# KhutornoyYaroslav/vcm-ts

Measured on AMD Instinct MI355X. Metric: encoded frames/sec at 1920x1080 GOP-32, higher is better.
Workload: dtype f32 (fp16x3 split-MFMA, fp32 accumulate)

## Files before the change

### include/dcvc_hip.h

```cpp
#ifndef DCVC_HIP_H
#define DCVC_HIP_H

#include <stdint.h>

#ifdef __cplusplus
extern "C" {
#endif

#define DCVC_OK 0
#define DCVC_E_ARG (-1)
#define DCVC_E_LAUNCH (-2)
#define DCVC_E_RANGE (-3)

#define DCVC_STATUS_ACT_SATURATED 1

#define DCVC_MAX_SEG 3

#define DCVC_PREC_FP32 0
#define DCVC_PREC_FP16X3 1

typedef struct {
    const float *ptr;
    int32_t C;
    int32_t cs;
} dcvc_seg;

typedef struct {
    dcvc_seg seg[DCVC_MAX_SEG];
    int32_t nseg;
    int32_t N, Hin, Win;
    int32_t in_act;
    float in_slope;
    const float *wpack;
    const float *bpack;
    int32_t ks;
    int32_t stride;
    int32_t Cout;
    int32_t Cout_pad;
    float *out;
    int32_t out_cs;
    int32_t out_act;
    float out_slope;
    int32_t pixel_shuffle;
    const float *res;
    int32_t res_cs;
    const float *res_gate;
    const float *res2;
    int32_t res2_cs;
    int32_t precision;
    int32_t *status;
    float *chan_partial;
    int32_t tile_row0;
    int32_t tile_rows;
    int32_t pair_taps;
} dcvc_conv_args;

int32_t dcvc_conv_tile_rows(int32_t ks, int32_t stride);

int32_t dcvc_conv_chan_partial_parts(int32_t ks, int32_t stride, int32_t Hout, int32_t Wout);
int dcvc_channel_mean_finish(const float *chan_partial, int32_t parts, int32_t row_stride, float *mean, int32_t N,
                             int32_t C, int32_t HW, void *stream);

int64_t dcvc_conv_pack_size(int32_t Cout, int32_t ks, int32_t nseg, const int32_t *seg_C, int32_t *cout_pad);

int dcvc_conv_pack_weights(const float *w, const float *b, int32_t Cout, int32_t ks, int32_t nseg,
                           const int32_t *seg_C, int32_t pixel_shuffle, int32_t precision, float *wpack,
                           float *bpack);

int64_t dcvc_conv_pack_size_paired(int32_t Cout, int32_t Cin, int32_t *cout_pad);
int dcvc_conv_pack_weights_paired(const float *w, const float *b, int32_t Cout, int32_t Cin, float *wpack, float *bpack);

int dcvc_conv2d(const dcvc_conv_args *a, void *stream);

int64_t dcvc_conv_small_pack_bytes(int32_t Cout, int32_t ks, int32_t nseg, const int32_t *seg_C);
int dcvc_conv_small_pack_weights(const float *w, const float *b, int32_t Cout, int32_t ks, int32_t nseg,
                                 const int32_t *seg_C, void *wpack, float *bpack);
int dcvc_conv2d_small(const dcvc_conv_args *a, void *stream);

int64_t dcvc_conv_k32_pack_bytes(int32_t Cout, int32_t ks, int32_t nseg, const int32_t *seg_C, int32_t *cout_pad);
int dcvc_conv_k32_pack_weights(const float *w, const float *b, int32_t Cout, int32_t ks, int32_t nseg,
                               const int32_t *seg_C, int32_t pixel_shuffle, void *wpack, float *bpack);
int dcvc_conv2d_k32(const dcvc_conv_args *a, void *stream);
int dcvc_conv_k32_set_waves(int32_t waves);

int dcvc_warp(const float *src, int32_t src_cs, const float *flow, int32_t flow_cs, float *out, int32_t out_cs,
              int32_t N, int32_t H, int32_t W, int32_t C, void *stream);
int dcvc_up2(const float *src, int32_t src_cs, float *out, int32_t out_cs, float *out2, int32_t out2_cs,
             int32_t N, int32_t H, int32_t W, int32_t C, float scale, void *stream);
int dcvc_down2(const float *src, int32_t src_cs, float *out, int32_t out_cs, int32_t N, int32_t H, int32_t W,
               int32_t C, float scale, int32_t avgpool_order, void *stream);
int dcvc_maxpool2(const float *src, int32_t src_cs, float *out, int32_t out_cs, int32_t N, int32_t H, int32_t W,
                  int32_t C, void *stream);
int dcvc_copy_channels(const float *src, int32_t src_cs, float *out, int32_t out_cs, int64_t npix, int32_t C,
                       void *stream);
int dcvc_nchw_to_nhwc(const float *src, float *out, int32_t out_cs, int32_t N, int32_t C, int32_t H, int32_t W,
                      void *stream);
int dcvc_nhwc_to_nchw(const float *src, int32_t src_cs, float *out, int32_t N, int32_t C, int32_t H, int32_t W,
                      int32_t clamp01, void *stream);

int dcvc_channel_mean(const float *src, int32_t src_cs, float *mean, float *scratch, int32_t N, int32_t HW,
                      int32_t C, void *stream);
int dcvc_se_gate(const float *mean, const float *w1, const float *w2, float *gate, int32_t N, int32_t C,
                 int32_t Cr, void *stream);

int dcvc_scale_channels(const float *src, int32_t src_cs, float *out, int32_t out_cs, const float *q_basic,
// ... 60 lines not shown
```

### vcm_ts_amd/csrc/conv_mfma.hip

```cpp
#include <hip/hip_runtime.h>
#include <stdint.h>
#include <stdlib.h>
#include <string.h>
#include <vector>

#include "dcvc_hip.h"
#include "kernel_common.h"

namespace {

constexpr int LDK = 20;


struct ConvK {
    const float *seg_ptr[DCVC_MAX_SEG];
    int seg_C[DCVC_MAX_SEG];
    int seg_cs[DCVC_MAX_SEG];
    int nseg;
    int Hin, Win, Hout, Wout;
    int in_act;
    float in_slope;
    const float *wpack;
    const float *bpack;
    int Cout, Cout_pad;
    float *out;
    int out_cs;
    int out_act;
    float out_slope;
    int ps;
    const float *res;
    int res_cs;
    const float *res_gate;
    const float *res2;
    int res2_cs;
    int vec_epi;
    int *status;
    float *chan_partial;
    int ntx;
    int ty0, nty;
    int band_rows;
};

inline long dev_env_long(const char *name, long dflt) {
    const char *dev = getenv("DCVC_DEV");
    if (!dev || strcmp(dev, "1") != 0) return dflt;
    const char *v = getenv(name);
    return v ? atol(v) : dflt;
}


template <int KS, int S, int RPW, int NT, bool SPLIT, bool PAIR = false>
__global__ __launch_bounds__(256, 2) void conv_mfma(const ConvK a) {
    static_assert(!PAIR || (KS == 7 && S == 1 && SPLIT), "tap pairing is built for the 7x7 split-fp16 layers");
    constexpr int BH = 4 * RPW, BW = 32, BN = 32 * NT;
    constexpr int PH = (BH - 1) * S + KS, PW = (BW - 1) * S + KS, PAD = KS / 2;
    constexpr int T = PAIR ? KS * 4 : KS * KS;
    constexpr int TPS = PAIR ? 4 : (KS == 3 && S == 1) ? 9 : KS;
    constexpr int NST = T / TPS;
    constexpr int EPI_LD = BN + 4;
    constexpr int LDS_MAIN = PH * PW * LDK + TPS * 4 * BN * 4, LDS_EPI = 4 * 32 * EPI_LD, LDS_RED = 4 * BN;
    __shared__ __attribute__((aligned(16))) float lds[LDS_MAIN > LDS_EPI + LDS_RED ? LDS_MAIN : LDS_EPI + LDS_RED];
    float *patch = lds;
    float *wl = lds + PH * PW * LDK;

    const int tid = threadIdx.x, lane = tid & 63, wave = tid >> 6;
    const int nbn = a.Cout_pad / BN;
    const int nb = blockIdx.x % nbn, tx = blockIdx.x / nbn;
    if (tx >= a.ntx) return;
    const int ty = blockIdx.y + a.ty0;
    const int x0 = tx * BW, y0 = ty * BH, n0 = nb * BN, img = blockIdx.z;

    f32x16 acc[RPW][NT];
#pragma unroll
    for (int m = 0; m < RPW; ++m)
#pragma unroll
        for (int n = 0; n < NT; ++n)
#pragma unroll
            for (int r = 0; r < 16; ++r) acc[m][n][r] = 0.f;

    const int a_base = ((wave * RPW * S) * PW + (lane & 31) * S) * LDK + (lane >> 5) * 4;
    const int b_base = ((lane >> 5) * BN + (lane & 31)) * 4;
// ... 273 lines not shown
#pragma unroll
            for (int r = 0; r < 16; ++r) {
                const int ox = x0 + (r & 3) + 8 * (r >> 2) + 4 * hh;
                const size_t pix = a.ps ? ((size_t)(img * Ho + 2 * oy + dy) * Wo + 2 * ox + dx)
                                        : ((size_t)(img * Ho + oy) * Wo + ox);
                rv[r] = (a.res && ox < a.Wout) ? a.res[pix * a.res_cs + cf] : 0.f;
                rv2[r] = (a.res2 && ox < a.Wout) ? a.res2[pix * a.res2_cs + cf] : 0.f;
            }
#pragma unroll
            for (int r = 0; r < 16; ++r) {
                const int ox = x0 + (r & 3) + 8 * (r >> 2) + 4 * hh;
                if (ox >= a.Wout) continue;
                float v = acc[m][n][r] * inv_scale + bias;
                if (a.out_act == 1) v = act(v, a.out_slope);
                else if (a.out_act == 2) v = fminf(fmaxf(v, 0.f), 1.f);
                const size_t pix = a.ps ? ((size_t)(img * Ho + 2 * oy + dy) * Wo + 2 * ox + dx)
                                        : ((size_t)(img * Ho + oy) * Wo + ox);
                if (a.out_act == 3) {
                    const float mk = rv2[r] > 0.f ? 1.f : a.out_slope;
                    v = a.res ? __builtin_fmaf(v, mk, rv[r]) : v * mk;
                } else {
                    if (a.res) v = a.res_gate ? __builtin_fmaf(rv[r], gate, v) : v + rv[r];
                    if (a.res2) v = rv2[r] + v;
                }
                if (a.status) vmax = fmaxf(vmax, fabsf(v));
                a.out[pix * a.out_cs + cf] = v;
            }
        }
    }
    if (a.status && !(vmax <= ACT_LIMIT)) atomicOr(a.status, DCVC_STATUS_ACT_SATURATED);
}


template <int KS, int S, int RPW, int NT, bool PAIR = false>
int launch(ConvK &k, int N, hipStream_t st, int precision) {
    constexpr int BH = 4 * RPW, BN = 32 * NT;
    k.ntx = (k.Wout + 31) / 32;
    static const bool xcd_pad = dev_env_long("DCVC_XCD_PAD", 0) != 0;
    unsigned gx = (unsigned)(k.ntx * (k.Cout_pad / BN));
    if (xcd_pad && gx >= 8) gx = (gx + 7) & ~7u;
    k.nty = (k.Hout + BH - 1) / BH;
    if (k.ty0 < 0 || k.ty0 >= k.nty) return DCVC_E_ARG;
    const int rows = k.band_rows > 0 ? (k.band_rows < k.nty - k.ty0 ? k.band_rows : k.nty - k.ty0) : k.nty;
    dim3 grid(gx, (unsigned)rows, (unsigned)N);
    if (PAIR)
        hipLaunchKernelGGL((conv_mfma<KS, S, RPW, NT, true, PAIR>), grid, dim3(256), 0, st, k);
    else if (precision == DCVC_PREC_FP16X3)
        hipLaunchKernelGGL((conv_mfma<KS, S, RPW, NT, true>), grid, dim3(256), 0, st, k);
    else
        hipLaunchKernelGGL((conv_mfma<KS, S, RPW, NT, false>), grid, dim3(256), 0, st, k);
    RET_LAUNCH();
}

}

extern "C" int64_t dcvc_conv_pack_size(int32_t Cout, int32_t ks, int32_t nseg, const int32_t *seg_C, int32_t *cout_pad) {
    if (Cout <= 0 || nseg <= 0 || nseg > DCVC_MAX_SEG || (ks != 1 && ks != 3 && ks != 7)) return DCVC_E_ARG;
    int chunks = 0;
    for (int s = 0; s < nseg; ++s) chunks += (seg_C[s] + MFMA_KC - 1) / MFMA_KC;
    const int cp = round_up(Cout, 32);
    if (cout_pad) *cout_pad = cp;
    return (int64_t)chunks * ks * ks * 4 * cp * 4;
}

extern "C" int dcvc_conv_pack_weights(const float *w, const float *b, int32_t Cout, int32_t ks, int32_t nseg,
                                      const int32_t *seg_C, int32_t pixel_shuffle, int32_t precision, float *wpack,
                                      float *bpack) {
    if (precision != DCVC_PREC_FP32 && precision != DCVC_PREC_FP16X3) return DCVC_E_ARG;
    int32_t cp = 0;
    const int64_t total = dcvc_conv_pack_size(Cout, ks, nseg, seg_C, &cp);
    if (total < 0 || (pixel_shuffle && (Cout & 3))) return DCVC_E_ARG;
    const int T = ks * ks;
    int Cin = 0;
    for (int s = 0; s < nseg; ++s) Cin += seg_C[s];
    memset(wpack, 0, (size_t)total * sizeof(float));
    memset(bpack, 0, (size_t)cp * sizeof(float));
    const int Cq = Cout / 4;
    _Float16 *base = (_Float16 *)wpack;
    int cg = 0, cin0 = 0;
    for (int s = 0; s < nseg; ++s) {
        for (int c0 = 0; c0 < seg_C[s]; c0 += MFMA_KC, ++cg) {
            for (int t = 0; t < T; ++t)
// ... 29 lines not shown
    int32_t cp = 0;
    const int64_t total = dcvc_conv_pack_size_paired(Cout, Cin, &cp);
    if (total < 0 || !w || !wpack || !bpack) return DCVC_E_ARG;
    memset(wpack, 0, (size_t)total * sizeof(float));
    memset(bpack, 0, (size_t)cp * sizeof(float));
    _Float16 *base = (_Float16 *)wpack;
    bool clamped = false;
    for (int ky = 0; ky < 7; ++ky)
        for (int kx = 0; kx < 7; ++kx) {
            const int step = ky * 4 + (kx >> 1), h = kx & 1;
            for (int c = 0; c < Cin; ++c)
                for (int n = 0; n < Cout; ++n) {
                    float sv = w[((size_t)n * Cin + c) * 49 + ky * 7 + kx] * WGT_SCALE;
                    if (!(fabsf(sv) <= F16_MAX)) { clamped = true; sv = sv > 0.f ? F16_MAX : -F16_MAX; }
                    const SplitF16 p = split_f16(sv);
                    base[mfma_wpack_f16(0, 28, step, 8 * h + c, cp, n, 0)] = p.hi;
                    base[mfma_wpack_f16(0, 28, step, 8 * h + c, cp, n, 1)] = p.lo;
                }
        }
    for (int n = 0; n < Cout; ++n) bpack[n] = b ? b[n] : 0.f;
    return clamped ? DCVC_E_RANGE : DCVC_OK;
}

static int tile_rows(int ks, int stride) { return stride == 2 ? 4 : 8; }

extern "C" int32_t dcvc_conv_tile_rows(int32_t ks, int32_t stride) { return tile_rows(ks, stride); }

extern "C" int32_t dcvc_conv_chan_partial_parts(int32_t ks, int32_t stride, int32_t Hout, int32_t Wout) {
    if (Hout <= 0 || Wout <= 0 || (stride != 1 && stride != 2)) return DCVC_E_ARG;
    const int bh = tile_rows(ks, stride);
    return ((Wout + 31) / 32) * ((Hout + bh - 1) / bh);
}

extern "C" int dcvc_conv2d(const dcvc_conv_args *a, void *stream) {
    if (!conv_args_ok(a)) return DCVC_E_ARG;
    if (a->stride != 1 && a->stride != 2) return DCVC_E_ARG;
    if (a->precision != DCVC_PREC_FP32 && a->precision != DCVC_PREC_FP16X3) return DCVC_E_ARG;
    if (a->Cout_pad % 32 || a->Cout > a->Cout_pad || (a->pixel_shuffle && (a->Cout & 3))) return DCVC_E_ARG;
    if (a->out_act < 0 || a->out_act > 3) return DCVC_E_ARG;
    if (a->out_act == 3 && (!a->res2 || a->res_gate || a->chan_partial || a->pixel_shuffle)) return DCVC_E_ARG;
    ConvK k;
    memset(&k, 0, sizeof(k));
    copy_conv_args_full(k, a);
    k.Hin = a->Hin;
    k.Win = a->Win;
    const int pad = a->ks / 2;
    k.Hout = (a->Hin + 2 * pad - a->ks) / a->stride + 1;
    k.Wout = (a->Win + 2 * pad - a->ks) / a->stride + 1;
    k.vec_epi = vec_epilogue_ok(a);
    if (a->chan_partial && (!k.vec_epi || a->pixel_shuffle)) return DCVC_E_ARG;
    hipStream_t st = (hipStream_t)stream;
    const bool wide = (a->Cout_pad % 64) == 0;
    const int key = a->ks * 10 + a->stride;
    if (a->stride == 1 && !a->pair_taps && !a->chan_partial && a->tile_rows <= 0) {
        const long wgs8 = (long)((k.Wout + 31) / 32) * ((k.Hout + 7) / 8) * (a->Cout_pad / (wide ? 64 : 32)) * a->N;
        static const long rows4_below = dev_env_long("DCVC_ROWS4_WGS", 384);
        if (wgs8 < rows4_below) {
            if (a->ks == 3) return wide ? launch<3, 1, 1, 2>(k, a->N, st, a->precision) : launch<3, 1, 1, 1>(k, a->N, st, a->precision);
            if (a->ks == 7) return wide ? launch<7, 1, 1, 2>(k, a->N, st, a->precision) : launch<7, 1, 1, 1>(k, a->N, st, a->precision);
            if (a->ks == 1) return wide ? launch<1, 1, 1, 2>(k, a->N, st, a->precision) : launch<1, 1, 1, 1>(k, a->N, st, a->precision);
        }
    }
    switch (key) {
        case 11: return wide ? launch<1, 1, 2, 2>(k, a->N, st, a->precision) : launch<1, 1, 2, 1>(k, a->N, st, a->precision);
        case 12: return wide ? launch<1, 2, 1, 2>(k, a->N, st, a->precision) : launch<1, 2, 1, 1>(k, a->N, st, a->precision);
        case 31:
            return wide ? launch<3, 1, 2, 2>(k, a->N, st, a->precision) : launch<3, 1, 2, 1>(k, a->N, st, a->precision);
        case 32: return wide ? launch<3, 2, 1, 2>(k, a->N, st, a->precision) : launch<3, 2, 1, 1>(k, a->N, st, a->precision);
        case 71:
            if (a->pair_taps) {
                if (a->nseg != 1 || a->seg[0].C > 8 || a->precision != DCVC_PREC_FP16X3 || a->pixel_shuffle) return DCVC_E_ARG;
                return wide ? launch<7, 1, 2, 2, true>(k, a->N, st, a->precision) : launch<7, 1, 2, 1, true>(k, a->N, st, a->precision);
            }
            return wide ? launch<7, 1, 2, 2>(k, a->N, st, a->precision) : launch<7, 1, 2, 1>(k, a->N, st, a->precision);
        default: return DCVC_E_ARG;
    }
}
```

### vcm_ts_amd/csrc/conv_small.hip

```cpp
#include <hip/hip_runtime.h>
#include <stdint.h>
#include <string.h>

#include "dcvc_hip.h"
#include "kernel_common.h"

namespace {

constexpr int KC = 16;

struct SmallK {
    const float *seg_ptr[DCVC_MAX_SEG];
    int seg_C[DCVC_MAX_SEG];
    int seg_cs[DCVC_MAX_SEG];
    int nseg;
    int H, W;
    int in_act;
    float in_slope;
    const char *wpack;
    const float *bpack;
    int Cout;
    float *out;
    int out_cs, out_act;
    float out_slope;
// ... 185 lines not shown

extern "C" int dcvc_conv_small_pack_weights(const float *w, const float *b, int32_t Cout, int32_t ks, int32_t nseg,
                                            const int32_t *seg_C, void *wpack, float *bpack) {
    const int64_t total = dcvc_conv_small_pack_bytes(Cout, ks, nseg, seg_C);
    if (total < 0 || !w || !wpack || !bpack) return DCVC_E_ARG;
    const int T = ks * ks;
    int Cin = 0;
    for (int s = 0; s < nseg; ++s) Cin += seg_C[s];
    memset(wpack, 0, (size_t)total);
    for (int n = 0; n < 16; ++n) bpack[n] = (b && n < Cout) ? b[n] : 0.f;
    _Float16 *base = (_Float16 *)wpack;
    int status = DCVC_OK, cg = 0, cin0 = 0;
    for (int s = 0; s < nseg; ++s) {
        for (int c0 = 0; c0 < seg_C[s]; c0 += KC, ++cg)
            for (int t = 0; t < T; ++t)
                for (int cc = 0; cc < KC && c0 + cc < seg_C[s]; ++cc)
                    for (int n = 0; n < Cout; ++n) {
                        float sv = w[((size_t)n * Cin + cin0 + c0 + cc) * T + t] * WGT_SCALE;
                        if (!(fabsf(sv) <= F16_MAX)) { status = DCVC_E_RANGE; sv = sv > 0.f ? F16_MAX : -F16_MAX; }
                        const SplitF16 p = split_f16(sv);
                        const size_t blk = ((size_t)cg * T + t) * 4;
                        base[((blk + (cc >> 3)) * 16 + n) * 8 + (cc & 7)] = p.hi;
                        base[((blk + 2 + (cc >> 3)) * 16 + n) * 8 + (cc & 7)] = p.lo;
                    }
        cin0 += seg_C[s];
    }
    return status;
}

extern "C" int dcvc_conv2d_small(const dcvc_conv_args *a, void *stream) {
    if (!conv_args_ok(a)) return DCVC_E_ARG;
    if (a->out_act < 0 || a->out_act > 2) return DCVC_E_ARG;
    if (a->tile_rows > 0) return DCVC_E_ARG;
    if (a->Cout <= 0 || a->Cout > 16 || (a->ks != 3 && a->ks != 7) || a->stride != 1 || a->pixel_shuffle || a->res_gate ||
        a->res2 || a->chan_partial || a->precision != DCVC_PREC_FP16X3 || a->N <= 0)
        return DCVC_E_ARG;
    SmallK k;
    memset(&k, 0, sizeof(k));
    copy_conv_args(k, a);
    k.H = a->Hin, k.W = a->Win;
    dim3 grid((unsigned)((a->Win + 31) / 32), (unsigned)((a->Hin + 7) / 8), (unsigned)a->N);
    if (a->ks == 7)
        hipLaunchKernelGGL(conv_small<7>, grid, dim3(256), 0, (hipStream_t)stream, k);
    else
        hipLaunchKernelGGL(conv_small<3>, grid, dim3(256), 0, (hipStream_t)stream, k);
    RET_LAUNCH();
}
```

### vcm_ts_amd/csrc/kernel_common.h

```cpp
#ifndef DCVC_KERNEL_COMMON_H
#define DCVC_KERNEL_COMMON_H

#include <hip/hip_runtime.h>
#include <stdint.h>

#include "dcvc_hip.h"

typedef float f32x16 __attribute__((ext_vector_type(16)));
typedef float f32x4 __attribute__((ext_vector_type(4)));
typedef _Float16 f16x8 __attribute__((ext_vector_type(8)));
typedef _Float16 f16x4 __attribute__((ext_vector_type(4)));

namespace {

#define RET_LAUNCH() return hipGetLastError() == hipSuccess ? DCVC_OK : DCVC_E_LAUNCH
inline unsigned nblk(int64_t n, int b) { return (unsigned)((n + b - 1) / b); }
inline int round_up(int v, int m) { return (v + m - 1) / m * m; }
inline bool aligned16(const void *p, int cs) { return p == nullptr || ((((uintptr_t)p) & 15) == 0 && (cs & 3) == 0); }

constexpr float ACT_SCALE = 8.f;
constexpr float WGT_SCALE = 64.f;
constexpr float F16_MAX = 65504.f;
constexpr float ACT_LIMIT = F16_MAX / ACT_SCALE;

__device__ __forceinline__ float act(float v, float slope) { return v > 0.f ? v : v * slope; }

__device__ __forceinline__ int32_t scale_index(float s, const float *edges) {
    int lo = 0;
#pragma unroll
    for (int step = 128; step >= 1; step >>= 1)
        if (edges[lo + step - 1] <= s) lo += step;
    return lo;
}

struct SplitF16 {
    _Float16 hi, lo;
};
__host__ __device__ inline SplitF16 split_f16(float sv) {
    const _Float16 hi = (_Float16)sv;
    return {hi, (_Float16)(sv - (float)hi)};
}

__host__ __device__ inline int ps_packed_channel(int n, int Cq) { return (n & 3) * Cq + (n >> 2); }
__host__ __device__ inline int ps_source_channel(int np, int Cq) { return (np % Cq) * 4 + np / Cq; }

constexpr int MFMA_KC = 16;
__host__ __device__ inline size_t mfma_wpack_f32(int cg, int T, int t, int cc, int cp, int np) {
    const int kq = cc >> 2, j = cc & 3;
    return ((((size_t)cg * T + t) * 4 + kq) * cp + np) * 4 + j;
}
__host__ __device__ inline size_t mfma_wpack_f16(int cg, int T, int t, int cc, int cp, int np, int lo) {
// ... 58 lines not shown
```

### vcm_ts_amd/engine.py

```python
from __future__ import annotations

import ctypes as C
import math

import numpy as np
import torch

from . import lib

_raw_stream = getattr(torch._C, "_cuda_getCurrentRawStream", None) or (lambda idx: torch.cuda.current_stream(idx).cuda_stream)


def _r4(c):
    return (c + 3) // 4 * 4


class View:

    __slots__ = ("base", "N", "H", "W", "C", "cs", "coff", "ptr")

    def __init__(self, base: torch.Tensor, C_: int, coff: int = 0, geom=None):
        self.base = base
        if geom is None:
            assert base.dim() == 4 and base.dtype == torch.float32 and base.is_contiguous()
# ... 29 lines not shown
    @property
    def HW(self):
        return self.H * self.W

    def __repr__(self):
        return f"View(N={self.N},H={self.H},W={self.W},C={self.C},cs={self.cs},coff={self.coff})"


class PackedConv:
    __slots__ = ("w", "b", "ks", "Cout", "Cout_pad", "seg_C", "ps", "version", "precision", "weight", "bias",
                 "cin_slice", "key", "small", "k32", "paired", "host", "job")


class Engine:
    def __init__(self, device, precision=None):
        import os

        self.precision = precision or os.environ.get("DCVC_PRECISION", "fp32")
        if self.precision not in lib.PRECISIONS:
            raise ValueError(f"precision must be one of {sorted(lib.PRECISIONS)}")
        self.device = torch.device(device)
        if self.device.type != "cuda":
            raise RuntimeError("the HIP engine needs a GPU device (no CPU fallback exists)")
        self._dev_index = self.device.index if self.device.index is not None else torch.cuda.current_device()
        self.L = lib.hip()
        self.bufs = {}
        self.packs = {}
        self._dev_packs = []
        self._plan = None
        self.calls = 0
        self.profile = None
        self.profile_detail = None
        self.profile_hbm = None
        self.tape = None
        self._edges = {}
        self._status = None
        dev = os.environ.get("DCVC_DEV") == "1"
        sw = lambda name, default: os.environ.get(name, default) if dev else default
        self.use_small = sw("DCVC_SMALL", "1") != "0"
        self.use_k32 = sw("DCVC_K32", "1") != "0"
        self.use_pairs = sw("DCVC_PAIR_TAPS", "1") != "0"
        self.k32_everywhere = False
        self.k32_sizes = tuple(int(k) for k in sw("DCVC_K32_SIZES", "3").split(","))
        self.range_check = os.environ.get("DCVC_RANGE_CHECK", "1") == "1"
        self.guard_outputs = True
        self.wgrad_split = os.environ.get("DCVC_WGRAD_SPLIT", "1") != "0"
        self.wgrad_side_stream = sw("DCVC_WGRAD_SIDE", "1") != "0"

    def stream(self):
        return C.c_void_p(_raw_stream(self._dev_index))

    def _store(self, scratch=False):
        return self.bufs if (self.tape is None or scratch) else self.tape.arena

    def buf(self, name, N, H, W, C_, cs=None, zero=False) -> View:
        cs = cs or _r4(C_)
        key = (name, N, H, W, cs)
        store = self._store()
        t = store.get(key)
        if t is None:
            t = (torch.zeros if zero else torch.empty)((N, H, W, cs), dtype=torch.float32, device=self.device)
            store[key] = t
        return View(t, C_)

    def status_word(self) -> torch.Tensor:
        if self._status is None:
# ... 221 lines not shown

    def _repacked(self, pk: PackedConv, variant) -> PackedConv:
        q = getattr(pk, variant, None)
        if q is None or q.version != pk.version:
            q = self._pack_host(variant, pk.key, pk.weight, pk.bias, pk.seg_C, pk.ps, pk.cin_slice, pk.version)
            setattr(pk, variant, q)
        return q

    def pair_capable(self, pk: PackedConv, stride) -> bool:
        return (self.precision == "fp16x3" and self.tape is None and self.use_pairs and getattr(pk, "host", False)
                and pk.ks == 7 and stride == 1 and len(pk.seg_C) == 1 and pk.seg_C[0] <= 8 and not pk.ps and pk.Cout > 16)

    def k32_capable(self, pk: PackedConv, stride, out: View, res, res2, gate, srcs=()) -> bool:
        if not (self.precision == "fp16x3" and self.tape is None and self.use_k32 and getattr(pk, "host", False)):
            return False
        cfin = pk.Cout // 4 if pk.ps else pk.Cout
        al = lambda v: v is None or (v.ptr % 16 == 0 and v.cs % 4 == 0)
        covered = (pk.ks in self.k32_sizes and stride == 1 and all(c % 32 == 0 for c in pk.seg_C) and cfin % 4 == 0
                   and al(out) and al(res) and al(res2) and (gate is None or gate.data_ptr() % 16 == 0)
                   and all(al(s) for s in srcs) and out.H * out.W < (1 << 24)
                   and all(v is None or v.cs * 4 < (1 << 24) for v in (out, res, res2, *srcs)))
        if not covered or self.k32_everywhere:
            return covered
        m = 2 if pk.ps else 1
        tiles = ((out.H // m + 7) // 8) * ((out.W // m + 31) // 32)
        return pk.Cout_pad % 64 == 0 and tiles * (pk.Cout_pad // 64) >= 1000

    def small_capable(self, pk: PackedConv, stride, gate, res2, chan_partial) -> bool:
        return (self.precision == "fp16x3" and self.tape is None and self.use_small and getattr(pk, "host", False)
                and pk.Cout <= 16 and pk.ks in (3, 7)
                and stride == 1 and not pk.ps and gate is None and res2 is None and chan_partial is None)

    def conv(self, pk: PackedConv, srcs, out: View, stride=1, in_slope=None, out_slope=None, res: View = None,
             gate: torch.Tensor = None, res2: View = None, chan_partial: torch.Tensor = None, band=None):
        return self._conv_f32(pk, srcs, out, stride, in_slope, out_slope, res, gate, res2, chan_partial, band)

    def _launch_conv(self, launch, pk, s0, Ho, Wo, stride, res, res2, tag="", note=""):
        if self.profile is None:
            launch()
            return
        ev0, ev1 = self._bracket(launch)
        flops = 2.0 * s0.N * Ho * Wo * pk.Cout * sum(pk.seg_C) * pk.ks * pk.ks
        nout = s0.N * Ho * Wo * pk.Cout
        abytes = 4.0 * (s0.N * s0.H * s0.W * sum(pk.seg_C) + nout * (1 + (res is not None) + (res2 is not None))
                        + pk.Cout * sum(pk.seg_C) * pk.ks * pk.ks)
        self.profile.setdefault(f"conv{pk.ks}x{pk.ks}s{stride}{tag}", []).append((ev0, ev1, flops, abytes))
        if self.profile_detail is not None:
            self.profile_detail.append((ev0, ev1, flops, f"k{pk.ks}s{stride}{tag} {pk.seg_C}->{pk.Cout}{'ps' if pk.ps else ''} "
                                                         f"{s0.H}x{s0.W}", note))

    @staticmethod
    def _bracket(launch):
        ev0, ev1 = torch.cuda.Event(enable_timing=True), torch.cuda.Event(enable_timing=True)
        ev0.record()
        launch()
        ev1.record()
        return ev0, ev1

    def chan_partial_buf(self, name, pk: PackedConv, out: View, stride=1):
        parts = int(self.L.dcvc_conv_chan_partial_parts(pk.ks, stride, out.H, out.W))
        if parts <= 0:
            raise lib.KernelError("conv_chan_partial_parts")
        return self.fbuf(name + ".chan_partial", out.N * parts * pk.Cout_pad), parts

    def _conv_f32(self, pk: PackedConv, srcs, out: View, stride=1, in_slope=None, out_slope=None, res: View = None,
                  gate: torch.Tensor = None, res2: View = None, chan_partial: torch.Tensor = None, band=None):
        a = lib.ConvArgs()
        assert len(srcs) == len(pk.seg_C)
        s0 = srcs[0]
        for i, (s, c) in enumerate(zip(srcs, pk.seg_C)):
            assert s.C == c and (s.N, s.H, s.W) == (s0.N, s0.H, s0.W), (s, c)
            a.seg[i].ptr, a.seg[i].C, a.seg[i].cs = s.ptr, s.C, s.cs
        a.nseg, a.N, a.Hin, a.Win = len(srcs), s0.N, s0.H, s0.W
        a.in_act, a.in_slope = (0, 0.0) if in_slope is None else (1, in_slope)
        small = band is None and self.small_capable(pk, stride, gate, res2, chan_partial)
        k32 = not small and not isinstance(out_slope, tuple) and self.k32_capable(pk, stride, out, res, res2, gate, srcs)
        paired = not small and not k32 and self.pair_capable(pk, stride)
        wq = self._repacked(pk, "small" if small else ("k32" if k32 else "paired")) if (small or k32 or paired) else pk
        a.pair_taps = int(paired)
        a.wpack, a.bpack = wq.w.data_ptr(), wq.b.data_ptr()
        a.ks, a.stride, a.Cout, a.Cout_pad = pk.ks, stride, pk.Cout, wq.Cout_pad
        pad = pk.ks // 2
        Ho = (s0.H + 2 * pad - pk.ks) // stride + 1
        Wo = (s0.W + 2 * pad - pk.ks) // stride + 1
        m = 2 if pk.ps else 1
        cfin = pk.Cout // 4 if pk.ps else pk.Cout
        assert (out.N, out.H, out.W, out.C) == (s0.N, Ho * m, Wo * m, cfin), (out, Ho, Wo, cfin)
        a.out, a.out_cs = out.ptr, out.cs
        if isinstance(out_slope, tuple):
            assert out_slope[0] == "mask" and res2 is not None and not (small or k32)
            a.out_act, a.out_slope = 3, float(out_slope[1])
        else:
            a.out_act, a.out_slope = (0, 0.0) if out_slope is None else ((2, 0.0) if out_slope == "clamp01" else (1, out_slope))
        a.pixel_shuffle = int(pk.ps)
        a.precision = pk.precision
        if res is not None:
            assert (res.N, res.H, res.W, res.C) == (out.N, out.H, out.W, out.C)
            a.res, a.res_cs = res.ptr, res.cs
        if gate is not None:
            a.res_gate = gate.data_ptr()
        if res2 is not None:
            assert (res2.N, res2.H, res2.W, res2.C) == (out.N, out.H, out.W, out.C)
            a.res2, a.res2_cs = res2.ptr, res2.cs
        if (self.range_check or k32) and self.precision == "fp16x3" and self.guard_outputs:
            a.status = self.status_word().data_ptr()
        if chan_partial is not None:
            a.chan_partial = chan_partial.data_ptr()
        if band is not None:
            a.tile_row0, a.tile_rows = int(band[0]), int(band[1])
        fn, what = (self.L.dcvc_conv2d_small, "conv2d_small") if small else (
            (self.L.dcvc_conv2d_k32, "conv2d_k32") if k32 else (self.L.dcvc_conv2d, "conv2d"))
        note = ""
        if self.profile_detail is not None:
            note = (f"{pk.key[0][1] if isinstance(pk.key[0], tuple) and len(pk.key[0]) > 1 else pk.key[0]}"
                    f" in_act={in_slope} out_act={out_slope} in_cs={[s.cs for s in srcs]} out_cs={out.cs}"
                    f" res={None if res is None else res.cs} gate={gate is not None} res2={None if res2 is None else res2.cs}"
                    f" chan_sums={chan_partial is not None}")
        self._launch_conv(lambda: lib.check(fn(C.byref(a), self.stream()), what), pk, s0, Ho, Wo, stride, res, res2,
                          "small" if small else ("k32" if k32 else ""), note)
        self.calls += 1
        self._rec("conv", pk, tuple(srcs), out, stride, in_slope, out_slope, res, gate, res2)
        return out

    def _hbm(self, kernel, shape, abytes, launch):
        if self.profile_hbm is None:
            return launch()
        ev0, ev1 = self._bracket(launch)
        self.profile_hbm.setdefault((kernel, shape), []).append((ev0, ev1, float(abytes)))

    def collect_profile_hbm(self):
        torch.cuda.synchronize(self.device)
        out = []
        for (kernel, shape), v in (self.profile_hbm or {}).items():
            ms = sum(r[0].elapsed_time(r[1]) for r in v)
            by = sum(r[2] for r in v)
            out.append({"kernel": kernel, "shape": shape, "launches": len(v), "avg_us": round(ms / len(v) * 1e3, 2),
                        "algorithmic_bytes": int(by / len(v)), "tb_per_s": round(by / (ms * 1e-3) / 1e12, 3) if ms > 0 else None})
        return out

    def collect_profile(self):
        torch.cuda.synchronize(self.device)
        return {k: {"flops": sum(r[2] for r in v), "bytes": sum(r[3] for r in v),
                    "ms": sum(r[0].elapsed_time(r[1]) for r in v), "launches": len(v)}
                for k, v in (self.profile or {}).items()}
# ... 160 lines not shown
```

### vcm_ts_amd/lib.py

```python
from __future__ import annotations

import ctypes as C
import os

HERE = os.path.dirname(os.path.abspath(__file__))
CSRC = os.path.join(HERE, "csrc")


class LibraryMissing(RuntimeError):
    pass


class KernelError(RuntimeError):
    pass


def _load(name):
    path = os.environ.get("DCVC_HIP_LIB") if name == "libdcvc_hip.so" and os.environ.get("DCVC_HIP_LIB") else \
        os.path.join(CSRC, name)
    if not os.path.exists(path):
        raise LibraryMissing(f"{path} not built; run `make -C {CSRC}` (no CPU fallback exists)")
    return C.CDLL(path)


# ... 6 lines not shown
        L = _load("libdcvc_rans.so")
        L.dcvc_rans_encoder_create.restype = C.c_void_p
        L.dcvc_rans_encoder_destroy.argtypes = [C.c_void_p]
        L.dcvc_rans_encoder_reset.argtypes = [C.c_void_p]
        L.dcvc_rans_encoder_encode_with_indexes.argtypes = [C.c_void_p, C.c_void_p, C.c_void_p, C.c_int64, C.c_void_p,
                                                            C.c_int32, C.c_int32, C.c_void_p, C.c_void_p]
        L.dcvc_rans_encoder_flush_bound.argtypes = [C.c_void_p]
        L.dcvc_rans_encoder_flush_bound.restype = C.c_int64
        L.dcvc_rans_encoder_flush.argtypes = [C.c_void_p, C.c_void_p, C.c_int64]
        L.dcvc_rans_encoder_flush.restype = C.c_int64
        L.dcvc_rans_decoder_create.restype = C.c_void_p
        L.dcvc_rans_decoder_destroy.argtypes = [C.c_void_p]
        L.dcvc_rans_decoder_set_stream.argtypes = [C.c_void_p, C.c_char_p, C.c_int64]
        L.dcvc_rans_decoder_decode_stream.argtypes = [C.c_void_p, C.c_void_p, C.c_int64, C.c_void_p, C.c_int32,
                                                      C.c_int32, C.c_void_p, C.c_void_p, C.c_void_p]
        L.dcvc_pmf_to_quantized_cdf.argtypes = [C.c_void_p, C.c_int32, C.c_int32, C.c_void_p]
        _rans = L
    return _rans


class Seg(C.Structure):
    _fields_ = [("ptr", C.c_void_p), ("C", C.c_int32), ("cs", C.c_int32)]


class ConvArgs(C.Structure):
    _fields_ = [
        ("seg", Seg * 3), ("nseg", C.c_int32), ("N", C.c_int32), ("Hin", C.c_int32), ("Win", C.c_int32),
        ("in_act", C.c_int32), ("in_slope", C.c_float), ("wpack", C.c_void_p), ("bpack", C.c_void_p),
        ("ks", C.c_int32), ("stride", C.c_int32), ("Cout", C.c_int32), ("Cout_pad", C.c_int32),
        ("out", C.c_void_p), ("out_cs", C.c_int32), ("out_act", C.c_int32), ("out_slope", C.c_float),
        ("pixel_shuffle", C.c_int32), ("res", C.c_void_p), ("res_cs", C.c_int32), ("res_gate", C.c_void_p),
        ("res2", C.c_void_p), ("res2_cs", C.c_int32), ("precision", C.c_int32), ("status", C.c_void_p),
        ("chan_partial", C.c_void_p), ("tile_row0", C.c_int32), ("tile_rows", C.c_int32), ("pair_taps", C.c_int32),
    ]


class DualPriorArgs(C.Structure):
    _fields_ = [
        ("y", C.c_void_p), ("y_cs", C.c_int32), ("fusion", C.c_void_p), ("fusion_cs", C.c_int32),
        ("spatial", C.c_void_p), ("spatial_cs", C.c_int32), ("params", C.c_void_p), ("params_cs", C.c_int32),
        ("y_hat", C.c_void_p), ("y_q", C.c_void_p), ("y_res", C.c_void_p), ("scales_hat", C.c_void_p),
        ("sym", C.c_void_p), ("idx", C.c_void_p), ("out", C.c_void_p), ("out_cs", C.c_int32),
        ("q_basic", C.c_void_p), ("q_scale", C.c_void_p), ("N", C.c_int32), ("H", C.c_int32), ("W", C.c_int32),
        ("C", C.c_int32), ("step", C.c_int32), ("idx_edges", C.c_void_p), ("forced_q", C.c_void_p),
        ("q_map", C.c_void_p),
    ]


class ConvBwdArgs(C.Structure):
    _fields_ = [
        ("dout", C.c_void_p), ("dout_cs", C.c_int32), ("out", C.c_void_p), ("out_cs", C.c_int32),
        ("res", C.c_void_p), ("res_cs", C.c_int32), ("gate", C.c_void_p), ("res2", C.c_void_p), ("res2_cs", C.c_int32),
        ("dres", C.c_void_p), ("dres_cs", C.c_int32), ("dres2", C.c_void_p), ("dres2_cs", C.c_int32),
        ("dpre", C.c_void_p), ("dpre_cs", C.c_int32), ("zs", C.c_int32), ("Hd", C.c_int32), ("Wd", C.c_int32),
        ("N", C.c_int32), ("Ho", C.c_int32), ("Wo", C.c_int32), ("Cout", C.c_int32), ("pixel_shuffle", C.c_int32),
        ("act", C.c_int32), ("slope", C.c_float),
    ]


class WgradArgs(C.Structure):
    _fields_ = [
        ("x", C.c_void_p), ("x_cs", C.c_int32), ("C", C.c_int32), ("in_act", C.c_int32), ("in_slope", C.c_float),
        ("dpre", C.c_void_p), ("dpre_cs", C.c_int32), ("zs", C.c_int32), ("Hd", C.c_int32), ("Wd", C.c_int32),
        ("N", C.c_int32), ("Hin", C.c_int32), ("Win", C.c_int32), ("Ho", C.c_int32), ("Wo", C.c_int32),
        ("Cout", C.c_int32), ("ks", C.c_int32), ("stride", C.c_int32), ("dw", C.c_void_p), ("Cin_total", C.c_int32),
        ("cin_offset", C.c_int32), ("scratch", C.c_void_p), ("scratch_floats", C.c_int64), ("overwrite", C.c_int32),
# ... 15 lines not shown
        ("y_hat", C.c_void_p), ("dout", C.c_void_p), ("dout_cs", C.c_int32), ("dy_res", C.c_void_p),
        ("dscales_hat", C.c_void_p), ("dparams", C.c_void_p), ("dparams_cs", C.c_int32),
        ("dspatial", C.c_void_p), ("dspatial_cs", C.c_int32), ("dy", C.c_void_p), ("dy_cs", C.c_int32),
        ("dfusion", C.c_void_p), ("dfusion_cs", C.c_int32), ("dq_plane", C.c_void_p),
        ("q_basic", C.c_void_p), ("q_scale", C.c_void_p), ("N", C.c_int32), ("H", C.c_int32), ("W", C.c_int32),
        ("C", C.c_int32), ("step", C.c_int32),
    ]


class ColorCoeffs(C.Structure):
    _fields_ = [(n, C.c_float) for n in ("y_off", "c_off", "y_scale", "c_scale", "crr", "cgb", "cgr", "cbb", "kr", "kg", "kb",
                                         "icb", "icr", "y_range", "c_range")] + \
               [(n, C.c_int32) for n in ("max_code", "bit_depth", "siting", "matrix", "range")]


class RoiBox(C.Structure):
    _fields_ = [(n, C.c_int32) for n in ("x1", "y1", "x2", "y2", "cls")]


class RoiClassRec(C.Structure):
    _fields_ = [("border", C.c_int32), ("shrink", C.c_int32), ("feather", C.c_float * 64)]


PRECISIONS = {"fp32": 0, "fp16x3": 1}

_hip = None
i32, i64, f32, vp = C.c_int32, C.c_int64, C.c_float, C.c_void_p

_SIGS = {
    "dcvc_conv2d": [C.POINTER(ConvArgs), vp],
    "dcvc_conv_pack_weights": [vp, vp, i32, i32, i32, vp, i32, i32, vp, vp],
    "dcvc_conv_pack_weights_paired": [vp, vp, i32, i32, vp, vp],
    "dcvc_conv2d_small": [C.POINTER(ConvArgs), vp],
    "dcvc_conv_small_pack_weights": [vp, vp, i32, i32, i32, vp, vp, vp],
    "dcvc_conv2d_k32": [C.POINTER(ConvArgs), vp],
    "dcvc_conv_k32_pack_weights": [vp, vp, i32, i32, i32, vp, i32, vp, vp],
    "dcvc_conv_k32_set_waves": [i32],
    "dcvc_warp": [vp, i32, vp, i32, vp, i32, i32, i32, i32, i32, vp],
    "dcvc_up2": [vp, i32, vp, i32, vp, i32, i32, i32, i32, i32, f32, vp],
    "dcvc_down2": [vp, i32, vp, i32, i32, i32, i32, i32, f32, i32, vp],
    "dcvc_maxpool2": [vp, i32, vp, i32, i32, i32, i32, i32, vp],
    "dcvc_copy_channels": [vp, i32, vp, i32, i64, i32, vp],
    "dcvc_nchw_to_nhwc": [vp, vp, i32, i32, i32, i32, i32, vp],
    "dcvc_nhwc_to_nchw": [vp, i32, vp, i32, i32, i32, i32, i32, vp],
    "dcvc_channel_mean": [vp, i32, vp, vp, i32, i32, i32, vp],
    "dcvc_se_gate": [vp, vp, vp, vp, i32, i32, i32, vp],
    "dcvc_channel_mean_finish": [vp, i32, i32, vp, i32, i32, i32, vp],
    "dcvc_scale_channels": [vp, i32, vp, i32, vp, vp, i32, i32, i32, i32, vp],
    "dcvc_scale_channels_map": [vp, i32, vp, i32, vp, vp, i32, i32, i32, i32, vp, i32, i32, vp],
    "dcvc_round_symbols": [vp, i32, vp, i32, vp, i32, i32, i32, i32, vp],
    "dcvc_symbols_to_nhwc": [vp, vp, i32, i32, i32, i32, i32, vp],
    "dcvc_scale_indexes": [vp, vp, i64, vp, vp],
    "dcvc_dual_prior_enc": [C.POINTER(DualPriorArgs), vp],
    "dcvc_dual_prior_dec_index": [C.POINTER(DualPriorArgs), vp],
    "dcvc_dual_prior_dec_apply": [C.POINTER(DualPriorArgs), vp],
    "dcvc_build_scale_cdfs": [vp, i32, i32, vp, vp, vp, vp],
    "dcvc_build_factorized_cdfs": [vp, i32, vp, vp, vp, vp],
    "dcvc_scale_bits": [vp, vp, vp, vp, i32, i32, i64, vp],
    "dcvc_factorized_bits": [vp, i32, vp, vp, vp, i32, i32, i32, vp],
    "dcvc_sq_err": [vp, i32, vp, i32, vp, vp, i32, i32, i32, vp],
    "dcvc_conv_pack_weights_dev": [vp, vp, i32, i32, i32, i32, vp, i32, i32, i32, i32, vp, vp, vp],
    "dcvc_pack_plan_create": [C.POINTER(PackJob), i32, C.POINTER(C.c_void_p)],
    "dcvc_pack_plan_run": [vp, vp],
    "dcvc_pack_plan_destroy": [vp],
    "dcvc_conv_bwd_prologue": [C.POINTER(ConvBwdArgs), vp],
    "dcvc_conv_wgrad": [C.POINTER(WgradArgs), vp],
# ... 109 lines not shown
```

Before: 42.31.

## Add larger conv tile shapes selected by workgroup count heuristic

Adds a pick_tile heuristic that picks 128-wide Cout tiles for stride-2 3x3 fp16x3 convs and 16-row tiles for 7x7 fp16x3 narrow convs once the grid has enough workgroups. It also exposes an explicit tile_shape override, a query for the chosen shape and an occupancy query. The larger tiles aim to improve weight and input reuse per workgroup, at the cost of fewer workgroups and possibly lower occupancy. Two new template instantiations (FAST_ONLY) are compiled for the fp16x3-only paths.

New measurement: 42.57, median of 6. No clear change (+0.6%).

```diff
diff --git a/include/dcvc_hip.h b/include/dcvc_hip.h
--- a/include/dcvc_hip.h
+++ b/include/dcvc_hip.h
@@ -53,6 +53,7 @@
     int32_t tile_row0;
     int32_t tile_rows;
     int32_t pair_taps;
+    int32_t tile_shape;
 } dcvc_conv_args;
 
 int32_t dcvc_conv_tile_rows(int32_t ks, int32_t stride);
@@ -71,6 +72,8 @@
 int dcvc_conv_pack_weights_paired(const float *w, const float *b, int32_t Cout, int32_t Cin, float *wpack, float *bpack);
 
 int dcvc_conv2d(const dcvc_conv_args *a, void *stream);
+int32_t dcvc_conv2d_tile_shape(const dcvc_conv_args *a);
+int32_t dcvc_conv_tile_residency(int32_t ks, int32_t stride, int32_t tile_shape, int32_t pair_taps);
 
 int64_t dcvc_conv_small_pack_bytes(int32_t Cout, int32_t ks, int32_t nseg, const int32_t *seg_C);
 int dcvc_conv_small_pack_weights(const float *w, const float *b, int32_t Cout, int32_t ks, int32_t nseg,
diff --git a/vcm_ts_amd/csrc/conv_mfma.hip b/vcm_ts_amd/csrc/conv_mfma.hip
--- a/vcm_ts_amd/csrc/conv_mfma.hip
+++ b/vcm_ts_amd/csrc/conv_mfma.hip
@@ -41,12 +41,7 @@
     int band_rows;
 };
 
-inline long dev_env_long(const char *name, long dflt) {
-    const char *dev = getenv("DCVC_DEV");
-    if (!dev || strcmp(dev, "1") != 0) return dflt;
-    const char *v = getenv(name);
-    return v ? atol(v) : dflt;
-}
+constexpr long ROWS16_WGS = 1000, S2C128_WGS = 256;
 
 
 template <int KS, int S, int RPW, int NT, bool SPLIT, bool PAIR = false>
@@ -386,8 +381,9 @@
 }
 
 
-template <int KS, int S, int RPW, int NT, bool PAIR = false>
+template <int KS, int S, int RPW, int NT, bool PAIR = false, bool FAST_ONLY = false>
 int launch(ConvK &k, int N, hipStream_t st, int precision) {
+    if (FAST_ONLY && precision != DCVC_PREC_FP16X3) return DCVC_E_ARG;
     constexpr int BH = 4 * RPW, BN = 32 * NT;
     k.ntx = (k.Wout + 31) / 32;
     static const bool xcd_pad = dev_env_long("DCVC_XCD_PAD", 0) != 0;
@@ -401,7 +397,7 @@
         hipLaunchKernelGGL((conv_mfma<KS, S, RPW, NT, true, PAIR>), grid, dim3(256), 0, st, k);
     else if (precision == DCVC_PREC_FP16X3)
         hipLaunchKernelGGL((conv_mfma<KS, S, RPW, NT, true>), grid, dim3(256), 0, st, k);
-    else
+    else if constexpr (!FAST_ONLY)
         hipLaunchKernelGGL((conv_mfma<KS, S, RPW, NT, false>), grid, dim3(256), 0, st, k);
     RET_LAUNCH();
 }
@@ -497,13 +493,75 @@
     return ((Wout + 31) / 32) * ((Hout + bh - 1) / bh);
 }
 
+static int pick_tile(const dcvc_conv_args *a, int Hout, int Wout) {
+    const bool wide = (a->Cout_pad % 64) == 0;
+    const bool fast = a->precision == DCVC_PREC_FP16X3;
+    const bool whole = !a->chan_partial && a->tile_rows <= 0;
+    if (a->tile_shape != 0 && !whole) return DCVC_E_ARG;
+    const long ntx = (Wout + 31) / 32;
+    if (a->stride == 2) {
+        int bn = wide ? 64 : 32;
+        if (a->tile_shape != 0) {
+            bn = a->tile_shape;
+            if ((bn != 32 && bn != 64 && bn != 128) || a->Cout_pad % bn || (bn == 128 && !(fast && a->ks == 3))) return DCVC_E_ARG;
+        } else if (whole && fast && a->ks == 3 && a->Cout_pad % 128 == 0) {
+            static const long c128_from = dev_env_long("DCVC_S2C128_WGS", S2C128_WGS);
+            if (ntx * ((Hout + 3) / 4) * (a->Cout_pad / 128) * a->N >= c128_from) bn = 128;
+        }
+        return bn;
+    }
+    int rows = 8;
+    if (a->tile_shape != 0) {
+        rows = a->tile_shape;
+        if (rows != 4 && rows != 8 && rows != 16) return DCVC_E_ARG;
+        if (rows == 4 && a->pair_taps) return DCVC_E_ARG;
+        if (rows == 16 && !(fast && a->ks == 7 && !a->pair_taps)) return DCVC_E_ARG;
+    } else if (whole) {
+        const long wgs8 = ntx * ((Hout + 7) / 8) * (a->Cout_pad / (wide ? 64 : 32)) * a->N;
+        static const long rows4_below = dev_env_long("DCVC_ROWS4_WGS", 384);
+        static const long rows16_from = dev_env_long("DCVC_ROWS16_WGS", ROWS16_WGS);
+        if (!a->pair_taps && wgs8 < rows4_below) rows = 4;
+        else if (fast && !wide && a->ks == 7 && !a->pair_taps && ntx * ((Hout + 15) / 16) * (a->Cout_pad / 32) * a->N >= rows16_from)
+            rows = 16;
+    }
+    return rows;
+}
+
+static bool conv2d_args_ok(const dcvc_conv_args *a) {
+    if (!conv_args_ok(a)) return false;
+    if (a->stride != 1 && a->stride != 2) return false;
+    if (a->precision != DCVC_PREC_FP32 && a->precision != DCVC_PREC_FP16X3) return false;
+    if (a->Cout_pad % 32 || a->Cout > a->Cout_pad || (a->pixel_shuffle && (a->Cout & 3))) return false;
+    if (a->out_act < 0 || a->out_act > 3) return false;
+    if (a->out_act == 3 && (!a->res2 || a->res_gate || a->chan_partial || a->pixel_shuffle)) return false;
+    return true;
+}
+
+extern "C" int32_t dcvc_conv_tile_residency(int32_t ks, int32_t stride, int32_t tile_shape, int32_t pair_taps) {
+    const void *fn = nullptr;
+    const int key = ks * 10000 + stride * 1000 + tile_shape;
+    if (pair_taps) {
+        if (key == 71008) fn = (const void *)conv_mfma<7, 1, 2, 1, true, true>;
+    } else {
+        if (key == 71016) fn = (const void *)conv_mfma<7, 1, 4, 1, true>;
+        if (key == 71008) fn = (const void *)conv_mfma<7, 1, 2, 1, true>;
+        if (key == 31008) fn = (const void *)conv_mfma<3, 1, 2, 1, true>;
+        if (key == 32128) fn = (const void *)conv_mfma<3, 2, 1, 4, true>;
+        if (key == 32064) fn = (const void *)conv_mfma<3, 2, 1, 2, true>;
+    }
+    int n = 0;
+    if (!fn || hipOccupancyMaxActiveBlocksPerMultiprocessor(&n, fn, 256, 0) != hipSuccess) return DCVC_E_ARG;
+    return n;
+}
+
+extern "C" int32_t dcvc_conv2d_tile_shape(const dcvc_conv_args *a) {
+    if (!conv2d_args_ok(a)) return DCVC_E_ARG;
+    const int pad = a->ks / 2;
+    return pick_tile(a, (a->Hin + 2 * pad - a->ks) / a->stride + 1, (a->Win + 2 * pad - a->ks) / a->stride + 1);
+}
+
 extern "C" int dcvc_conv2d(const dcvc_conv_args *a, void *stream) {
-    if (!conv_args_ok(a)) return DCVC_E_ARG;
-    if (a->stride != 1 && a->stride != 2) return DCVC_E_ARG;
-    if (a->precision != DCVC_PREC_FP32 && a->precision != DCVC_PREC_FP16X3) return DCVC_E_ARG;
-    if (a->Cout_pad % 32 || a->Cout > a->Cout_pad || (a->pixel_shuffle && (a->Cout & 3))) return DCVC_E_ARG;
-    if (a->out_act < 0 || a->out_act > 3) return DCVC_E_ARG;
-    if (a->out_act == 3 && (!a->res2 || a->res_gate || a->chan_partial || a->pixel_shuffle)) return DCVC_E_ARG;
+    if (!conv2d_args_ok(a)) return DCVC_E_ARG;
     ConvK k;
     memset(&k, 0, sizeof(k));
     copy_conv_args_full(k, a);
@@ -516,27 +574,31 @@
     if (a->chan_partial && (!k.vec_epi || a->pixel_shuffle)) return DCVC_E_ARG;
     hipStream_t st = (hipStream_t)stream;
     const bool wide = (a->Cout_pad % 64) == 0;
-    const int key = a->ks * 10 + a->stride;
-    if (a->stride == 1 && !a->pair_taps && !a->chan_partial && a->tile_rows <= 0) {
-        const long wgs8 = (long)((k.Wout + 31) / 32) * ((k.Hout + 7) / 8) * (a->Cout_pad / (wide ? 64 : 32)) * a->N;
-        static const long rows4_below = dev_env_long("DCVC_ROWS4_WGS", 384);
-        if (wgs8 < rows4_below) {
-            if (a->ks == 3) return wide ? launch<3, 1, 1, 2>(k, a->N, st, a->precision) : launch<3, 1, 1, 1>(k, a->N, st, a->precision);
-            if (a->ks == 7) return wide ? launch<7, 1, 1, 2>(k, a->N, st, a->precision) : launch<7, 1, 1, 1>(k, a->N, st, a->precision);
-            if (a->ks == 1) return wide ? launch<1, 1, 1, 2>(k, a->N, st, a->precision) : launch<1, 1, 1, 1>(k, a->N, st, a->precision);
-        }
-    }
-    switch (key) {
-        case 11: return wide ? launch<1, 1, 2, 2>(k, a->N, st, a->precision) : launch<1, 1, 2, 1>(k, a->N, st, a->precision);
-        case 12: return wide ? launch<1, 2, 1, 2>(k, a->N, st, a->precision) : launch<1, 2, 1, 1>(k, a->N, st, a->precision);
-        case 31:
-            return wide ? launch<3, 1, 2, 2>(k, a->N, st, a->precision) : launch<3, 1, 2, 1>(k, a->N, st, a->precision);
-        case 32: return wide ? launch<3, 2, 1, 2>(k, a->N, st, a->precision) : launch<3, 2, 1, 1>(k, a->N, st, a->precision);
-        case 71:
-            if (a->pair_taps) {
-                if (a->nseg != 1 || a->seg[0].C > 8 || a->precision != DCVC_PREC_FP16X3 || a->pixel_shuffle) return DCVC_E_ARG;
-                return wide ? launch<7, 1, 2, 2, true>(k, a->N, st, a->precision) : launch<7, 1, 2, 1, true>(k, a->N, st, a->precision);
-            }
+    const int tile = pick_tile(a, k.Hout, k.Wout);
+    if (tile < 0) return tile;
+    if (a->stride == 2) {
+        if (a->ks == 3) {
+            if (tile == 128) return launch<3, 2, 1, 4, false, true>(k, a->N, st, a->precision);
+            return tile == 64 ? launch<3, 2, 1, 2>(k, a->N, st, a->precision) : launch<3, 2, 1, 1>(k, a->N, st, a->precision);
+        }
+        if (a->ks == 1) return tile == 64 ? launch<1, 2, 1, 2>(k, a->N, st, a->precision) : launch<1, 2, 1, 1>(k, a->N, st, a->precision);
+        return DCVC_E_ARG;
+    }
+    if (a->pair_taps && a->ks == 7) {
+        if (a->nseg != 1 || a->seg[0].C > 8 || a->precision != DCVC_PREC_FP16X3 || a->pixel_shuffle) return DCVC_E_ARG;
+    }
+    if (tile == 4) {
+        if (a->ks == 3) return wide ? launch<3, 1, 1, 2>(k, a->N, st, a->precision) : launch<3, 1, 1, 1>(k, a->N, st, a->precision);
+        if (a->ks == 7) return wide ? launch<7, 1, 1, 2>(k, a->N, st, a->precision) : launch<7, 1, 1, 1>(k, a->N, st, a->precision);
+        if (a->ks == 1) return wide ? launch<1, 1, 1, 2>(k, a->N, st, a->precision) : launch<1, 1, 1, 1>(k, a->N, st, a->precision);
+        return DCVC_E_ARG;
+    }
+    if (tile == 16) return launch<7, 1, 4, 1, false, true>(k, a->N, st, a->precision);
+    switch (a->ks) {
+        case 1: return wide ? launch<1, 1, 2, 2>(k, a->N, st, a->precision) : launch<1, 1, 2, 1>(k, a->N, st, a->precision);
+        case 3: return wide ? launch<3, 1, 2, 2>(k, a->N, st, a->precision) : launch<3, 1, 2, 1>(k, a->N, st, a->precision);
+        case 7:
+            if (a->pair_taps) return wide ? launch<7, 1, 2, 2, true>(k, a->N, st, a->precision) : launch<7, 1, 2, 1, true>(k, a->N, st, a->precision);
             return wide ? launch<7, 1, 2, 2>(k, a->N, st, a->precision) : launch<7, 1, 2, 1>(k, a->N, st, a->precision);
         default: return DCVC_E_ARG;
     }
diff --git a/vcm_ts_amd/csrc/conv_small.hip b/vcm_ts_amd/csrc/conv_small.hip
--- a/vcm_ts_amd/csrc/conv_small.hip
+++ b/vcm_ts_amd/csrc/conv_small.hip
@@ -241,6 +241,7 @@
     if (!conv_args_ok(a)) return DCVC_E_ARG;
     if (a->out_act < 0 || a->out_act > 2) return DCVC_E_ARG;
     if (a->tile_rows > 0) return DCVC_E_ARG;
+    if (a->tile_shape != 0 && a->tile_shape != 8) return DCVC_E_ARG;
     if (a->Cout <= 0 || a->Cout > 16 || (a->ks != 3 && a->ks != 7) || a->stride != 1 || a->pixel_shuffle || a->res_gate ||
         a->res2 || a->chan_partial || a->precision != DCVC_PREC_FP16X3 || a->N <= 0)
         return DCVC_E_ARG;
diff --git a/vcm_ts_amd/csrc/kernel_common.h b/vcm_ts_amd/csrc/kernel_common.h
--- a/vcm_ts_amd/csrc/kernel_common.h
+++ b/vcm_ts_amd/csrc/kernel_common.h
@@ -3,6 +3,8 @@
 
 #include <hip/hip_runtime.h>
 #include <stdint.h>
+#include <stdlib.h>
+#include <string.h>
 
 #include "dcvc_hip.h"
 
@@ -17,6 +19,13 @@
 inline unsigned nblk(int64_t n, int b) { return (unsigned)((n + b - 1) / b); }
 inline int round_up(int v, int m) { return (v + m - 1) / m * m; }
 inline bool aligned16(const void *p, int cs) { return p == nullptr || ((((uintptr_t)p) & 15) == 0 && (cs & 3) == 0); }
+
+inline long dev_env_long(const char *name, long dflt) {
+    const char *dev = getenv("DCVC_DEV");
+    if (!dev || strcmp(dev, "1") != 0) return dflt;
+    const char *v = getenv(name);
+    return v ? atol(v) : dflt;
+}
 
 constexpr float ACT_SCALE = 8.f;
 constexpr float WGT_SCALE = 64.f;
diff --git a/vcm_ts_amd/engine.py b/vcm_ts_amd/engine.py
--- a/vcm_ts_amd/engine.py
+++ b/vcm_ts_amd/engine.py
@@ -85,6 +85,7 @@
         self.profile = None
         self.profile_detail = None
         self.profile_hbm = None
+        self.tile_log = None
         self.tape = None
         self._edges = {}
         self._status = None
@@ -372,8 +373,8 @@
                 and stride == 1 and not pk.ps and gate is None and res2 is None and chan_partial is None)
 
     def conv(self, pk: PackedConv, srcs, out: View, stride=1, in_slope=None, out_slope=None, res: View = None,
-             gate: torch.Tensor = None, res2: View = None, chan_partial: torch.Tensor = None, band=None):
-        return self._conv_f32(pk, srcs, out, stride, in_slope, out_slope, res, gate, res2, chan_partial, band)
+             gate: torch.Tensor = None, res2: View = None, chan_partial: torch.Tensor = None, band=None, tile_shape=0):
+        return self._conv_f32(pk, srcs, out, stride, in_slope, out_slope, res, gate, res2, chan_partial, band, tile_shape)
 
     def _launch_conv(self, launch, pk, s0, Ho, Wo, stride, res, res2, tag="", note=""):
         if self.profile is None:
@@ -404,7 +405,7 @@
         return self.fbuf(name + ".chan_partial", out.N * parts * pk.Cout_pad), parts
 
     def _conv_f32(self, pk: PackedConv, srcs, out: View, stride=1, in_slope=None, out_slope=None, res: View = None,
-                  gate: torch.Tensor = None, res2: View = None, chan_partial: torch.Tensor = None, band=None):
+                  gate: torch.Tensor = None, res2: View = None, chan_partial: torch.Tensor = None, band=None, tile_shape=0):
         a = lib.ConvArgs()
         assert len(srcs) == len(pk.seg_C)
         s0 = srcs[0]
@@ -448,8 +449,11 @@
             a.chan_partial = chan_partial.data_ptr()
         if band is not None:
             a.tile_row0, a.tile_rows = int(band[0]), int(band[1])
+        a.tile_shape = int(tile_shape)
         fn, what = (self.L.dcvc_conv2d_small, "conv2d_small") if small else (
             (self.L.dcvc_conv2d_k32, "conv2d_k32") if k32 else (self.L.dcvc_conv2d, "conv2d"))
+        if self.tile_log is not None and not (small or k32):
+            self.tile_log.append(int(self.L.dcvc_conv2d_tile_shape(C.byref(a))))
         note = ""
         if self.profile_detail is not None:
             note = (f"{pk.key[0][1] if isinstance(pk.key[0], tuple) and len(pk.key[0]) > 1 else pk.key[0]}"
diff --git a/vcm_ts_amd/lib.py b/vcm_ts_amd/lib.py
--- a/vcm_ts_amd/lib.py
+++ b/vcm_ts_amd/lib.py
@@ -62,6 +62,7 @@
         ("pixel_shuffle", C.c_int32), ("res", C.c_void_p), ("res_cs", C.c_int32), ("res_gate", C.c_void_p),
         ("res2", C.c_void_p), ("res2_cs", C.c_int32), ("precision", C.c_int32), ("status", C.c_void_p),
         ("chan_partial", C.c_void_p), ("tile_row0", C.c_int32), ("tile_rows", C.c_int32), ("pair_taps", C.c_int32),
+        ("tile_shape", C.c_int32),
     ]
 
 
@@ -143,6 +144,8 @@
     "dcvc_conv_pack_weights": [vp, vp, i32, i32, i32, vp, i32, i32, vp, vp],
     "dcvc_conv_pack_weights_paired": [vp, vp, i32, i32, vp, vp],
     "dcvc_conv2d_small": [C.POINTER(ConvArgs), vp],
+    "dcvc_conv2d_tile_shape": [C.POINTER(ConvArgs)],
+    "dcvc_conv_tile_residency": [i32, i32, i32, i32],
     "dcvc_conv_small_pack_weights": [vp, vp, i32, i32, i32, vp, vp, vp],
     "dcvc_conv2d_k32": [C.POINTER(ConvArgs), vp],
     "dcvc_conv_k32_pack_weights": [vp, vp, i32, i32, i32, vp, i32, vp, vp],
```
